# Luckick/EAGCN

Measured on AMD Instinct MI355X. Metric: molecules/sec fwd+bwd, 2-layer 5-view EAGCN, Tox21 batch, higher is better.
Workload: dtype f32 (bf16x3 split, fp32 accumulate): every fp32 operand leaves its producer as three bf16 planes, six v_mfma_f32_32x32x16_bf16 piece products per 16 k rebuild the fp32 product (csrc/gemm_bx3.hip); aggregation, BatchNorm, head, first layer fp32

## Files before the change

eagcn_amd/_lib.py:

```python
import ctypes as C
import os

_HERE = os.path.dirname(os.path.abspath(__file__))
LIB_PATH = os.path.join(_HERE, 'lib', 'libeagcn_hip.so')

MAX_VIEWS = 8
MAX_SEGS = 8
META_WORDS = 16
META_NLOG = 8
META_T, META_NMAX, META_NTILES, META_BAD_ADJ, META_BAD_REL, META_NEDGE, META_OVERFLOW, META_EDGE_OVERFLOW = range(8)
META_NBLK = 9
STRUCT_CONCATE, STRUCT_WEIGHTED = 0, 1

_fp = C.c_void_p


class Batch(C.Structure):
    _fields_ = [('B', C.c_int32), ('N', C.c_int32), ('K', C.c_int32), ('ldc', C.c_int32),
                ('T', C.c_int32), ('n_max', C.c_int32), ('n_tiles', C.c_int32),
                ('channels', C.c_int32 * MAX_VIEWS),
                ('code', _fp), ('deg_bn', _fp), ('nat', _fp), ('row0', _fp), ('tile0', _fp),
                ('meta', _fp), ('row_mol', _fp), ('row_loc', _fp), ('row_m', _fp), ('row_deg', _fp),
                ('tile_mol', _fp), ('row_info', _fp), ('tile_info', _fp),
                ('rel_vec', _fp * MAX_VIEWS), ('rel_c', C.c_int32 * MAX_VIEWS),
# ... 171 lines not shown
    'eagcn_index_build': (C.c_int, [_fp, C.POINTER(_fp), C.POINTER(Batch), _fp, _fp]),
    'eagcn_index_from_bonds': (C.c_int, [_fp, _fp, _fp, _fp, C.c_int64, C.POINTER(Batch), _fp, _fp]),
    'eagcn_index_rows': (C.c_int, [C.POINTER(Batch), _fp]),
    'eagcn_set_gemm_mode': (C.c_int, [C.c_int]),
    'eagcn_stream_wait_counter': (C.c_int, [_fp, C.c_uint32, _fp]),
    'eagcn_stream_signal_flag': (C.c_int, [_fp, _fp]),
    'eagcn_stream_wait_flag': (C.c_int, [_fp, C.c_double, _fp]),
    'eagcn_stream_wait_timeouts': (C.c_int, []),
    'eagcn_stream_wait_reset': (None, []),
    'eagcn_adam_step': (C.c_int, [_fp, _fp, _fp, _fp, C.c_int64, _fp, _fp, _fp, _fp]),
    'eagcn_grad_norm_workspace_bytes': (C.c_size_t, []),
    'eagcn_grad_norm': (C.c_int, [_fp, _fp, C.c_int64, _fp, C.c_int, _fp]),
    'eagcn_adam_step_clipped': (C.c_int, [_fp, _fp, _fp, _fp, C.c_int64, _fp, _fp, _fp, _fp, _fp, _fp, _fp]),
    'eagcn_agg_wants_bond_lists': (C.c_int, [C.c_int, C.c_int]),
    'eagcn_agg_wants_bond_lists_for': (C.c_int, [C.c_int, C.c_int, C.c_int]),
    'eagcn_bx3_used_splits': (C.c_int, [C.c_int, C.c_int, C.c_int, C.c_int]),
    'eagcn_set_bx3_wide': (C.c_int, [C.c_int]),
    'eagcn_set_top_bn_sums': (C.c_int, [C.c_int]),
    'eagcn_set_hidden_bn_sums': (C.c_int, [C.c_int]),
    'eagcn_hidden_bn_sums_taken': (C.c_long, [C.c_int]),
    'eagcn_set_first_layer_fused': (C.c_int, [C.c_int]),
    'eagcn_first_layer_fused_taken': (C.c_long, [C.c_int]),
    'eagcn_first_layer_fused_last': (None, [C.POINTER(C.c_int32)]),
    'eagcn_bx3_pair_used_splits': (C.c_int, [C.c_int] * 7),
    'eagcn_bx3_plane_elems': (C.c_size_t, [C.c_int, C.c_int]),
    'eagcn_bx3_split': (C.c_int, [_fp, C.c_int, C.c_int, _fp, C.c_size_t, C.c_int, C.c_int, _fp]),
    'eagcn_gemm_bx3': (C.c_int, [C.c_int, C.c_int, C.c_int, C.c_int, _fp, C.c_size_t, C.c_int, C.c_int, _fp, C.c_size_t, C.c_int, C.c_int,
                                 _fp, C.c_int, C.c_int, C.c_size_t, C.c_int, _fp]),
    'eagcn_gemm_bx3_pair': (C.c_int, [C.c_int, C.c_int, C.c_int, _fp, C.c_size_t, C.c_int, C.c_int, _fp, C.c_size_t, C.c_int, C.c_int, _fp, C.c_int,
                                      C.c_int, C.c_int, C.c_int, _fp, C.c_size_t, C.c_int, C.c_int, _fp, C.c_size_t, C.c_int, C.c_int, _fp, C.c_int,
                                      C.c_int, C.c_size_t, C.c_int, _fp]),
    'eagcn_pack_rows': (C.c_int, [C.POINTER(Batch), _fp, C.c_int, C.POINTER(Layout), _fp, _fp]),
    'eagcn_unpack_rows': (C.c_int, [C.POINTER(Batch), _fp, C.POINTER(Layout), _fp, _fp, C.c_int, _fp]),
    'eagcn_pad_rows': (C.c_int, [_fp, _fp, C.c_int, C.c_int, C.c_int, _fp, _fp]),
    'eagcn_gat_scratch_bytes': (C.c_size_t, [C.POINTER(Batch), C.c_int]),
    'eagcn_gat_forward': (C.c_int, [C.POINTER(Batch), C.POINTER(GatParams), _fp, _fp, _fp, _fp, _fp]),
    'eagcn_gat_backward': (C.c_int, [C.POINTER(Batch), C.POINTER(GatParams), _fp, _fp, _fp, _fp, _fp, _fp, _fp, _fp, _fp,
                                     C.c_size_t, _fp]),
    'eagcn_pool_scratch_bytes': (C.c_size_t, []),
    'eagcn_pool_attention_forward': (C.c_int, [C.POINTER(Batch), C.POINTER(PoolAtt), _fp, C.c_int, _fp, _fp, _fp]),
    'eagcn_pool_attention_backward': (C.c_int, [C.POINTER(Batch), C.POINTER(PoolAtt), _fp, C.c_int, _fp, _fp, _fp, C.c_size_t,
                                                _fp]),
    'eagcn_pool_mix_forward': (C.c_int, [C.POINTER(Batch), C.POINTER(Layout), _fp, C.c_int, _fp, _fp, _fp, _fp, C.c_int, _fp]),
    'eagcn_pool_mix_backward': (C.c_int, [C.POINTER(Batch), C.POINTER(Layout), _fp, C.c_int, _fp, _fp, _fp, _fp, C.c_int, _fp,
                                          _fp, _fp, _fp]),
    'eagcn_pool_reduce_forward': (C.c_int, [C.POINTER(Batch), _fp, C.c_int, C.c_int, C.c_int, _fp, _fp, _fp, _fp]),
# ... 157 lines not shown
```

eagcn_amd/build.py:

```python
import os
import shutil
import subprocess
import sys
from concurrent.futures import ThreadPoolExecutor

HERE = os.path.dirname(os.path.abspath(__file__))
CSRC = os.path.join(HERE, 'csrc')
LIBDIR = os.path.join(HERE, 'lib')
LIB = os.path.join(LIBDIR, 'libeagcn_hip.so')
HIP_SOURCES = ['index.hip', 'gemm.hip', 'gemm3.hip', 'gemm_bx3.hip', 'gemm_bx3w.hip', 'agg.hip', 'lagg.hip', 'lagg_in.hip', 'lagg_top.hip', 'lagg_dw.hip', 'gat.hip', 'pool.hip', 'layer.hip', 'readout.hip', 'head.hip', 'head2.hip', 'loss.hip', 'clip.hip', 'attr.hip', 'battr.hip', 'metrics.hip', 'reps.hip', 'embed.hip', 'knn.hip']
CPP_SOURCES = ['api.cpp']
HEADERS = ['common.h', 'kernels.h', 'lagg_kernel.h', 'gemm_x6.h', 'bx3.h', 'bx3_epi.h', os.path.join('..', '..', 'include', 'eagcn_hip.h')]
ARCH = 'gfx950'


def _hipcc():
    for cand in (shutil.which('hipcc'), '/opt/rocm/bin/hipcc'):
        if cand and os.path.exists(cand):
            return cand
    raise RuntimeError('hipcc not found: the EAGCN HIP library cannot be built')


def _newest(paths):
    return max(os.path.getmtime(p) for p in paths)


def needs_build():
    srcs = [os.path.join(CSRC, s) for s in HIP_SOURCES + CPP_SOURCES + HEADERS if os.path.exists(os.path.join(CSRC, s))]
    return (not os.path.exists(LIB)) or os.path.getmtime(LIB) < _newest(srcs)


def build_library(force=False, verbose=False):
    if not force and not needs_build():
# ... 38 lines not shown
```

eagcn_amd/csrc/kernels.h:

```cpp
#pragma once
#include "bx3.h"
#include "common.h"

namespace eagcn {

struct AggArgs {
    eagcn_batch bt;
    ViewCols vc;
    const float* src; int lds;
    float* dst; int ldd;
    const float* sig;
    const float* rsig;
    float* rscale;
    double* stats;
    int nchunk;
    int cpw = 1;
    int xcd = 0;
    bool w_rowm = false;
    bool w_gather = false;
    BxOut planes = {nullptr, 0, 0, 0};
    const float* bn_tab = nullptr; const float* bn_cc = nullptr; int bn_fp = 0;
    const float* w_aw = nullptr;
    int w_drop = 0; uint32_t w_thr = 0; float w_inv_keep = 1.0f; uint64_t w_seed = 0; const uint64_t* w_seed_dev = nullptr;
    const float* fx = nullptr; int fx_ld = 0; float* dw = nullptr; size_t dw_slab = 0; int dw_ny = 0;
};
struct DropArgs { int on; uint32_t thr; float inv_keep; uint64_t seed; const uint64_t* seed_dev; };
inline DropArgs drop_args(float p, bool training, uint64_t seed, const uint64_t* seed_dev) {
    const double thr = (double)p * 4294967296.0;
    return DropArgs{(training && p > 0.0f) ? 1 : 0, (uint32_t)(thr < 4294967295.0 ? thr : 4294967295.0), 1.0f / (1.0f - p), seed, seed_dev};
}
inline void agg_set_drop(AggArgs& a, const DropArgs& d) {
    a.w_drop = d.on; a.w_thr = d.thr; a.w_inv_keep = d.inv_keep; a.w_seed = d.seed; a.w_seed_dev = d.seed_dev;
}
int agg_grid_x(const eagcn_batch* b);
bool agg_ksplit(const eagcn_batch* b);
int launch_agg(AggArgs a, bool trans, hipStream_t s);
constexpr int LAGG_RB = 256;
constexpr int LAGG_MAXM = 16;
struct EdgeArgs;
int lagg_parts();
bool lagg_wfuse();
bool lagg_use(const eagcn_batch* b, int dir, bool absorbs_bn, const ViewCols* vc = nullptr);
bool lagg_wanted(int B, int N, int structure);
int lagg_block_rows(const eagcn_batch* b);
int lagg_slabs(const eagcn_batch* b);
int launch_lagg_fwd(AggArgs a, hipStream_t s);
int launch_lagg_bwd(AggArgs a, const EdgeArgs& e, hipStream_t s, bool edge = true);
int launch_lagg_bwd_input(const AggArgs& a, const EdgeArgs& e, dim3 grid, hipStream_t s);
int launch_lagg_bwd_top(const AggArgs& a, const EdgeArgs& e, dim3 grid, hipStream_t s);
int launch_lagg_bwd_dw(const AggArgs& a, const EdgeArgs& e, dim3 grid, hipStream_t s);
int lagg_bwd_grid_y(const eagcn_batch* b, const ViewCols& vc);

struct EdgeArgs {
    eagcn_batch bt;
    ViewCols vc;
    const float* dY; const float* Y; const float* P; int ld;
    const float* sig; const float* rsig; const float* rscale;
    double* datt;
    int atomic;
    int xcd = 0;
};
constexpr int EDGE_SLAB = 264;
constexpr int EDGE_COPIES = 8;
inline size_t edge_acc_bytes() { return align256((size_t)EDGE_COPIES * EAGCN_MAX_VIEWS * EDGE_SLAB * sizeof(double)); }
int edge_grid_x(const eagcn_batch* b);
int launch_agg_edge(AggArgs a, const EdgeArgs& e, hipStream_t s);

enum { BN_SC = 0, BN_SH, BN_MU, BN_INV };

struct ColMapD {
    int nseg;
    int w[EAGCN_MAX_SEGS], p[EAGCN_MAX_SEGS];
};
// ... 182 lines not shown
struct PlanAsk {
    bool has_dx = false;
    bool mol_grad = false;
    bool input_only = false;
    bool has_drain_out = false;
    bool top_sums = false;
    bool top_gather = false;
    bool dh_given = false;
    bool below = false;
};
struct LayerRoute {
    FwdProd fwd_prod = FWD_NONE; bool fwd_split_x = false;
    AggPath fwd_agg = AGG_DENSE, bwd_agg = AGG_DENSE;
    Bn2 bn2 = BN2_NONE;
    bool rows_first = false, rows_late = false;
    bool store_dh = false;
    EdgePath edge = EDGE_NONE; bool edge_atomic = false;
    BwdProd bwd_prod = BWD_NONE; bool bwd_split_x = false;
    bool bx_wide = false;
    bool carries_below = false;
    bool defer_drain = false;
    bool dh_given = false;
    bool dw_fused = false; int dw_ny = 0; bool dw_in_dp = false;
    bool bn2_staged() const { return bn2 >= BN2_STAGED_FROM_DH; }
    bool bwd_planes() const { return bwd_prod >= BWD_PLANES_PAIR && bwd_prod <= BWD_PLANES_DX; }
};
LayerRoute plan_layer(const eagcn_batch* b, const eagcn_layer_params* p, const eagcn_layer_bufs* w, const PlanAsk& ask);
int layer_backward_impl(const eagcn_batch* b, const eagcn_layer_params* p, const eagcn_layer_bufs* w, const float* dxout,
                        const float* dpad_row, float* dx, const eagcn_layer_grads* g, void* stream, const LayerRoute& r,
                        const LayerBwdOpts& o = LayerBwdOpts{});
int model_backward_input_packed(const eagcn_batch* b, const eagcn_model* m, const int64_t* size, void* saved, size_t saved_bytes,
                                void* scratch, size_t scratch_bytes, const float* dout, const float* dgraph_rep,
                                const eagcn_layer_grads* lg, const eagcn_head_grads* hg, float** dx0, void* stream, const char* who);
int launch_attr_dense(const eagcn_batch* b, const eagcn_layout* in, const float* acc, const float* x, const float* base, float* attr,
                      float* score, hipStream_t s);
int model_input_slot(const eagcn_batch* b, const eagcn_model* m, void* saved, size_t saved_bytes, float** x0, const char* who);
int layer_forward_impl(const eagcn_batch* b, const eagcn_layer_params* p, const eagcn_layer_bufs* w, void* stream, const LayerRoute& r,
                       bool prepacked, bool skip_apply = false, bool planes_only = false);
inline int check_reserved_null(const void* value, const char* who, const char* field) {
    EAGCN_CHECK_ARG(!value, "%s: %s is reserved and must be null", who, field);
    return EAGCN_OK;
}
int layer_apply_impl(const eagcn_batch* b, const eagcn_layer_params* p, const eagcn_layer_bufs* w, void* stream);
int pack_params_all(const eagcn_batch* b, const eagcn_layer_params* const* ps, void* const* packed,
                    const size_t* packed_bytes, int n, void* stream, const ZeroJob* zj = nullptr, const HandOff* ho = nullptr);
struct ReadoutBn {
// ... 22 lines not shown
```

eagcn_amd/csrc/lagg.hip:

```cpp
#include <stdlib.h>

#include <algorithm>

#include "common.h"
#include "kernels.h"
#include "lagg_kernel.h"

namespace eagcn {


static int lagg_cpw(const eagcn_batch& bt, const ViewCols& vc, bool trans);
static int lagg_policy() {
    static const int v = [] {
        const char* e = getenv("EAGCN_AGG");
        if (e && !strcmp(e, "lds")) return 1;
        if (e && !strcmp(e, "dense")) return 0;
        return 2;
    }();
    return v;
}
static int lagg_min_n() {
    static const int v = env_int("EAGCN_LAGG_MIN_N", 240);
    return v;
}
// ... 44 lines not shown
    static const int cpw_env = env_int("EAGCN_LAGG_CPW", 0);
    static const int cpw_bwd = env_int("EAGCN_LAGG_CPW_BWD", 1);
    int chunks, gy;
    lagg_extent(bt, vc, &chunks, &gy);
    const long wgs = (long)vc.K * chunks * gy;
    int per = (trans && !cpw_bwd) ? 1 : cpw_env > 0 ? cpw_env : (int)std::min<long>(trans ? 4 : 8, std::max<long>(1, wgs / 3072));
    return std::max(1, std::min(per, chunks));
}
static int lagg_grid(const AggArgs& a, dim3* grid, int* nchunk, int* cpw, bool trans) {
    int chunks, gy;
    lagg_extent(a.bt, a.vc, &chunks, &gy);
    *cpw = lagg_cpw(a.bt, a.vc, trans);
    *nchunk = cdiv(chunks, *cpw);
    *grid = dim3((unsigned)(a.vc.K * *nchunk), (unsigned)gy);
    return EAGCN_OK;
}

int lagg_bwd_grid_y(const eagcn_batch* b, const ViewCols& vc) {
    int chunks, gy;
    lagg_extent(*b, vc, &chunks, &gy);
    return gy;
}

int launch_lagg_fwd(AggArgs a, hipStream_t s) {
    if (a.bt.B == 0 || a.bt.T == 0) return EAGCN_OK;
    dim3 grid;
    int rc = lagg_grid(a, &grid, &a.nchunk, &a.cpw, false);
    if (rc) return rc;
    ProfScope ps(PROF_AGG, s);
    EdgeArgs e;
    memset(&e, 0, sizeof(e));
    if (a.cpw > 1) lagg_kernel<false, true><<<grid, 256, 0, s>>>(a, e);
    else lagg_kernel<false, false><<<grid, 256, 0, s>>>(a, e);
    EAGCN_LAUNCH_CHECK();
    return EAGCN_OK;
}

int launch_lagg_bwd(AggArgs a, const EdgeArgs& e, hipStream_t s, bool edge) {
    if (a.bt.B == 0 || a.bt.T == 0) return EAGCN_OK;
    EAGCN_CHECK_ARG(!edge || (e.atomic && e.datt), "lagg: the edge gradients leave through the shared accumulator slabs (EdgeArgs.atomic)");
    dim3 grid;
    int rc = lagg_grid(a, &grid, &a.nchunk, &a.cpw, true);
    if (rc) return rc;
    ProfScope ps(PROF_AGG, s);
    EAGCN_CHECK_ARG(!a.w_aw || a.bn_tab, "lagg: the upstream-gradient form needs the BatchNorm tables");
    EAGCN_CHECK_ARG(!a.w_rowm || a.bn_tab, "lagg: the row-mask staging needs the BatchNorm tables");
    if (!edge) {
        rc = launch_lagg_bwd_input(a, e, grid, s);
        if (rc) return rc;
    } else if (a.w_rowm) {
        rc = launch_lagg_bwd_top(a, e, grid, s);
        if (rc) return rc;
// ... 19 lines not shown
```

eagcn_amd/csrc/lagg_kernel.h:

```cpp
#pragma once

#include "common.h"
#include "kernels.h"

namespace eagcn {

constexpr int LG_CW = 32;
constexpr int LG_LPR = LG_CW / 4;
constexpr int LG_G = 256 / LG_LPR;
constexpr int LG_U = LAGG_RB / LG_G;
constexpr int LG_ECAP = 768;
constexpr int LG_EPT = LG_ECAP / 256;
constexpr bool LG_MERGE = true;
constexpr int LG_PJ_EARLY = 4;

__device__ __forceinline__ void lg_fma(float4& acc, float w, const float4& v) {
    acc.x = fmaf(w, v.x, acc.x); acc.y = fmaf(w, v.y, acc.y); acc.z = fmaf(w, v.z, acc.z); acc.w = fmaf(w, v.w, acc.w);
}
__device__ __forceinline__ void lg_add(float4& acc, const float4& v) { acc.x += v.x; acc.y += v.y; acc.z += v.z; acc.w += v.w; }
__device__ __forceinline__ float lg_dot(const float4& a, const float4& b) { return fmaf(a.x, b.x, fmaf(a.y, b.y, fmaf(a.z, b.z, a.w * b.w))); }
template <int CTRL>
__device__ __forceinline__ float lg_dpp(float v) {
    return __int_as_float(__builtin_amdgcn_update_dpp(0, __float_as_int(v), CTRL, 0xF, 0xF, true));
}
__device__ __forceinline__ float lg_gsum(float v) {
    v += lg_dpp<0xB1>(v); v += lg_dpp<0x4E>(v); v += lg_dpp<0x141>(v);
    return v;
}

struct LgLists {
    unsigned short nb[LG_ECAP];
    float w[LG_ECAP];
    unsigned char cd[LG_ECAP];
};
constexpr uint32_t LG_SLOW = 1u << 28;
constexpr uint32_t LG_OVF = 1u << 29;
constexpr int LG_NOVF = 32;

template <bool TRANS, bool MULTI, bool WFUSE = false, bool EDGE = true, bool CROWS = false, bool GATHER = false, bool DWF = false>
__global__ __launch_bounds__(256) __attribute__((amdgpu_waves_per_eu(3, 8))) void lagg_kernel(AggArgs a, EdgeArgs ed) {
    static_assert(!DWF || (TRANS && EDGE && !WFUSE), "the weight-gradient epilogue belongs to the plain transposed kernel with the edge gradients");
    static_assert(TRANS || !WFUSE, "the upstream-gradient form belongs to the transposed kernel");
    static_assert(TRANS || EDGE, "the forward has no edge gradients to drop");
    static_assert(!CROWS || WFUSE, "the row-mask staging is a form of the upstream-gradient staging");
    static_assert(!GATHER || (CROWS && EDGE && MULTI), "the per-molecule gather is a form of the row-mask staging with the edge gradients");
    constexpr bool TE = TRANS && EDGE;
    constexpr int NREC = TRANS ? 3 : 2;
    __shared__ float4 buf[LAGG_RB][LG_LPR];
    __shared__ float4 s_rec[LAGG_RB][NREC];
    __shared__ float4 s_ovf[LG_NOVF][NREC];
    __shared__ int s_novf;
    __shared__ __attribute__((aligned(16))) unsigned char s_lists_raw[TRANS ? 16 : sizeof(LgLists)];
    __shared__ float s_rs[TRANS ? LAGG_RB : 1];
    __shared__ float s_rd[TE ? LAGG_RB : 1];
    __shared__ unsigned char s_rm[LAGG_RB];
    __shared__ float4 s_S[LAGG_MAXM][LG_LPR];
    __shared__ float sig_s[256];
    __shared__ double st_s[TRANS ? 1 : 4][TRANS ? 1 : LG_LPR][8];
    __shared__ float4 s_bn[TRANS ? (WFUSE ? 4 : 3) : 1][LG_LPR];
    __shared__ double h_s[TE ? 264 : 1];
    static_assert(sizeof(LgLists) <= sizeof(float4) * LAGG_RB * 3, "lists alias the transposed record array");
    LgLists& L = *reinterpret_cast<LgLists*>(TRANS ? reinterpret_cast<unsigned char*>(&s_rec[0][0]) : s_lists_raw);
    const eagcn_batch& bt = a.bt;
    const int tid = threadIdx.x, lane = tid & 63, wave = tid >> 6;
// ... 200 lines not shown
#pragma unroll
                for (int i = 0; i < NREC; ++i) s_rec[tid][i] = rec[i];
            }
        };
        if constexpr (MULTI) {
            hdr_loads();
            if (nst > 0) list_loads();
            __syncthreads();
            lists_to_lds();
            __syncthreads();
            build_record();
            if constexpr (TRANS) __syncthreads();
            write_record();
        }
        for (int cc = cc_lo; cc < cc_hi; ++cc) {
        set_chunk(cc);
        asm volatile("" : "+v"(g));
        const bool bn_next = MULTI && TRANS && fuse_bn && tid < LG_CW;

        float4 v[LG_U], yv[TRANS ? LG_U : 1];
        float rmv[(CROWS && !EDGE) ? LG_U : 1];
        int ce = 0;
        if constexpr (GATHER) { const int cx = c0s - a.vc.off[k]; ce = ex0 + (cx < a.vc.width[k] ? cx : 0); }
#pragma unroll
        for (int u = 0; u < LG_U; ++u) {
            const int rc = min(g + LG_G * u, rows - 1);
            if constexpr (GATHER) v[u] = *reinterpret_cast<const float4*>(a.src + ((uint32_t)(m0 + s_rm[rc]) * (uint32_t)a.lds + (uint32_t)ce));
            else v[u] = *reinterpret_cast<const float4*>(a.src + (size_t)(R0 + rc) * a.lds + ((WFUSE && !CROWS) ? (col_ok ? col : 0) : c0s));
            if constexpr (TRANS) yv[u] = *reinterpret_cast<const float4*>(ed.Y + (size_t)(R0 + rc) * ed.ld + c0s);
            if constexpr (CROWS && !EDGE) rmv[u] = bt.row_m[R0 + rc];
        }
        if constexpr (!MULTI) {
            hdr_loads();
            if (nst > 0) list_loads();
        }
        uint32_t keep = 0xFFFFFFFFu;
        if constexpr (WFUSE) {
            if (a.w_drop) {
                keep = 0u;
                const uint32_t t16 = a.w_thr >> 16;
#pragma unroll
                for (int u = 0; u < LG_U; ++u) {
                    const uint64_t z = rng_u64(wseed, ((uint64_t)(R0 + g + LG_G * u) * a.bn_fp + c0s) >> 2);
                    const uint32_t lo = (uint32_t)z, hi = (uint32_t)(z >> 32);
                    keep |= ((lo & 0xFFFFu) >= t16 ? 1u : 0u) << (4 * u);
                    keep |= ((lo >> 16) >= t16 ? 2u : 0u) << (4 * u);
                    keep |= ((hi & 0xFFFFu) >= t16 ? 4u : 0u) << (4 * u);
                    keep |= ((hi >> 16) >= t16 ? 8u : 0u) << (4 * u);
                }
            }
        }
        __syncthreads();
        if (tid < LAGG_MAXM * LG_LPR) {
            float z;
            asm volatile("v_mov_b32 %0, 0" : "=v"(z));
            (&s_S[0][0])[tid] = make_float4(z, z, z, z);
        }
#pragma unroll
        for (int u = 0; u < LG_U; ++u) {
            const int rr = g + LG_G * u;
            const bool mine = rr < rows;
            if constexpr (TRANS) {
                if (fuse_bn) {
                    if constexpr (WFUSE) {
                        int lq = l;
                        asm volatile("" : "+v"(lq));
                        if constexpr (GATHER) {
                            if (c0s - a.vc.off[k] >= a.vc.width[k]) v[u] = make_float4(0.f, 0.f, 0.f, 0.f);
                        }
                        uint32_t mb;
                        {
                            const float4 bA = s_bn[0][lq], sh = s_bn[3][lq];
                            const uint32_t kb = keep >> (4 * u);
                            mb = ((yv[u].x * bA.x + sh.x > 0.0f) ? (kb & 1u) : 0u) | ((yv[u].y * bA.y + sh.y > 0.0f) ? (kb & 2u) : 0u) |
                                 ((yv[u].z * bA.z + sh.z > 0.0f) ? (kb & 4u) : 0u) | ((yv[u].w * bA.w + sh.w > 0.0f) ? (kb & 8u) : 0u);
                        }
                        asm volatile("" : "+v"(mb));
                        {
                            const float ik = a.w_drop ? a.w_inv_keep : 1.0f;
                            float wm = w_ave;
                            if constexpr (CROWS && !EDGE) wm = rmv[u];
                            if constexpr (CROWS && EDGE) wm = s_rs[rr] > 0.0f ? 1.0f : 0.0f;
// ... 136 lines not shown
            if constexpr (AHEAD) {
#pragma unroll
                for (int i = 0; i < NREC; ++i) nrec[i] = s_rec[min(g, rows - 1)][i];
            }
            const int nu = (rows + LG_G - 1) / LG_G;
#pragma unroll
            for (int u = 0; u < LG_U; ++u) {
                if (!DWF && u >= nu) break;
                const int rr = min(g + LG_G * u, rows - 1);
                const bool valid = g + LG_G * u < rows;
                if constexpr (!AHEAD) {
#pragma unroll
                    for (int i = 0; i < NREC; ++i) nrec[i] = s_rec[rr][i];
                }
                const float4 r0 = nrec[0], r1 = nrec[1], rl = nrec[NREC - 1];
                if (AHEAD && u + 1 < LG_U) {
#pragma unroll
                    for (int i = 0; i < NREC; ++i) nrec[i] = s_rec[min(rr + LG_G, rows - 1)][i];
                }
                const uint32_t srcs = __float_as_uint(TRANS ? rl.y : rl.z), meta = __float_as_uint(rl.w);
                const bool fast = valid && !(meta & LG_SLOW);
                any_slow = any_slow || (valid && (meta & LG_SLOW));
                const float4 self = buf[rr][l];
                const float4 S = s_S[(meta >> 24) & 15u][l];
                const float4 v0 = buf[srcs & 255u][l], v1 = buf[(srcs >> 8) & 255u][l], v2 = buf[(srcs >> 16) & 255u][l], v3 = buf[srcs >> 24][l];
                const float ws = TRANS ? r * rl.x : r1.x;
                const float wS = TRANS ? TINY : r1.y * TINY;
                float4 y;
                y.x = fmaf(r0.x, v0.x, fmaf(r0.y, v1.x, fmaf(r0.z, v2.x, fmaf(r0.w, v3.x, fmaf(ws, self.x, wS * S.x)))));
                y.y = fmaf(r0.x, v0.y, fmaf(r0.y, v1.y, fmaf(r0.z, v2.y, fmaf(r0.w, v3.y, fmaf(ws, self.y, wS * S.y)))));
                y.z = fmaf(r0.x, v0.z, fmaf(r0.y, v1.z, fmaf(r0.z, v2.z, fmaf(r0.w, v3.z, fmaf(ws, self.z, wS * S.z)))));
                y.w = fmaf(r0.x, v0.w, fmaf(r0.y, v1.w, fmaf(r0.z, v2.w, fmaf(r0.w, v3.w, fmaf(ws, self.w, wS * S.w)))));
                if constexpr (TE && LG_MERGE) {
                    const float4 pj = col_ok ? pjv[u] : make_float4(0.f, 0.f, 0.f, 0.f);
                    const uint32_t cds = __float_as_uint(rl.z);
                    const float g0 = lg_gsum(lg_dot(v0, pj)), g1 = lg_gsum(lg_dot(v1, pj)), g2 = lg_gsum(lg_dot(v2, pj)), g3 = lg_gsum(lg_dot(v3, pj));
                    const float gs = lg_gsum(lg_dot(self, pj));
                    const int e4 = l & 3;
                    const float hv = e4 == 0 ? r1.x : e4 == 1 ? r1.y : e4 == 2 ? r1.z : r1.w;
                    const float gv = e4 == 0 ? g0 : e4 == 1 ? g1 : e4 == 2 ? g2 : g3;
                    const uint32_t cv = (cds >> (8 * e4)) & 255u, sv = (srcs >> (8 * e4)) & 255u;
                    if (fast && l < 4 && hv != 0.0f && cv) atomicAdd(&h_s[cv], (double)hv * ((double)gv - (double)s_rd[sv]));
                    if (fast && l == 4) dr_acc += (double)rl.x * ((double)gs - (double)s_rd[rr]);
                }
                if (fast && (meta & LG_OVF)) {
                    const int slot = (int)(meta & 0xFFFFu);
// ... 177 lines not shown
```

eagcn_amd/csrc/layer.hip:

```cpp
#include <algorithm>

#include <stdlib.h>

#include "common.h"
#include "kernels.h"

namespace eagcn {

struct ParamPtrs {
    const float* att_w[EAGCN_MAX_VIEWS];
    const float* self_r[EAGCN_MAX_VIEWS];
    const float* W[EAGCN_MAX_VIEWS];
    const float* bias[EAGCN_MAX_VIEWS];
    const float* gamma[EAGCN_MAX_VIEWS];
    const float* beta[EAGCN_MAX_VIEWS];
    float* run_mean[EAGCN_MAX_VIEWS];
    float* run_var[EAGCN_MAX_VIEWS];
    const float* ave_w;
    int channels[EAGCN_MAX_VIEWS];
    const float* rel_vec[EAGCN_MAX_VIEWS];
    int rel_c[EAGCN_MAX_VIEWS];
};
__device__ __forceinline__ float att_logit(const ParamPtrs& pp, int k, int c) {
    if (!pp.rel_vec[k]) return pp.att_w[k][c - 1];
// ... 849 lines not shown
static Fp32Products layer_fp32_products(const eagcn_batch* b, const LayerDims& d, const LayerOperands& o, double work) {
    const int* T_dev = b->meta + EAGCN_META_T;
    Fp32Products q{GemmDesc{0, 1, b->T, d.fp, d.ld_in, o.x, d.ld_in, o.pk.WcatT, d.ld_in, o.P, d.fp, 1, 0, work},
                   GemmDesc{0, 0, b->T, d.fp, d.ld_in, o.x, d.ld_in, o.pk.Wcat, d.fp, o.P, d.fp, 1, 0, work},
                   GemmDesc{0, 1, b->T, d.ld_in, d.fp, o.dP, d.fp, o.pk.Wcat, d.fp, o.dx, d.ld_in, 1, 0, work},
                   GemmDesc{1, 0, d.ld_in, d.fp, b->T, o.x, d.ld_in, o.dP, d.fp, o.dWcat, d.fp, d.nsplit, d.wslab, work}};
    q.gp.M_dev = T_dev; q.gt.M_dev = T_dev; q.gx.M_dev = T_dev; q.gw.K_dev = T_dev;
    return q;
}

static bool sw_gemm3() { static const bool on = !env_flag("EAGCN_NO_GEMM3", false); return on; }
bool planes_only_enabled() { static const bool on = env_flag("EAGCN_PLANES_ONLY", true); return on; }
static bool bn_bwd_two_pass(bool weighted) {
    static const int force = getenv("EAGCN_BWD_STORE_DH") ? (env_flag("EAGCN_BWD_STORE_DH", false) ? 1 : 0) : -1;
    return force < 0 ? weighted : force == 0;
}
static bool gemm3_layer(int ld_in) {
    return sw_gemm3() && ld_in >= 128 && gemm_mode() != 2;
}
static int g_first_layer_fused = env_flag("EAGCN_FIRST_LAYER_FUSED", true) ? 1 : 0;
static long g_first_layer_fused_taken = 0;
static int32_t g_first_layer_fused_last[3] = {0, 0, 0};
static bool first_layer_fused_enabled() { return g_first_layer_fused != 0; }
static int g_hidden_bn_sums = env_flag("EAGCN_HIDDEN_BN_SUMS", true) ? 1 : 0;
static long g_hidden_bn_taken = 0;

static LayerRoute plan_layer(const eagcn_batch* b, const eagcn_layer_params* p, const eagcn_layer_bufs* w, const LayerDims& d,
                             const PlanAsk& ask) {
    LayerRoute r;
    const bool wt = p->structure == EAGCN_STRUCT_WEIGHTED;
    bool general = false;
    for (int k = 0; k < p->K; ++k) general = general || b->rel_vec[k] != nullptr;
    r.edge_atomic = !general;
    r.store_dh = !bn_bwd_two_pass(wt);
    if (b->T <= 0) return r;
    r.fwd_agg = fwd_agg_lagg(b, d.vc) ? AGG_LAGG : AGG_DENSE;
    float* const some_dx = reinterpret_cast<float*>(static_cast<uintptr_t>(4096));
    LayerScratch sc;
    carve_layer(w->scratch, b, d, true, &sc);
    if (w->packed) carve_packed(w->packed, d, &sc.pk);
    const LayerOperands o = layer_operands(w, sc, ask.has_dx ? some_dx : nullptr);
    const PlaneProducts bq = layer_plane_products(b, d, o);
    const Fp32Products gq = layer_fp32_products(b, d, o, 0.0);

    r.fwd_split_x = d.np && !w->x_planes;
    if (d.np && bx3_ok(bq.bp)) r.fwd_prod = FWD_PLANES;
    else if (!w->x) r.fwd_prod = FWD_REFUSED;
    else r.fwd_prod = (gemm3_layer(d.ld_in) && gemm3_ok(gq.gp)) ? FWD_BALANCED : FWD_TILED;

    const bool fuse_w = bn_bwd_two_pass(wt) && wt && lagg_wfuse();
    const bool absorbs = !bn_bwd_two_pass(wt) || (wt && lagg_wfuse());
    const bool lagg = ask.input_only ? lagg_use(b, 1, true) : (r.edge_atomic && lagg_use(b, 1, absorbs));
    r.bwd_agg = lagg ? AGG_LAGG : AGG_DENSE;
    if (ask.input_only && !p->training) {
        r.bn2 = !lagg ? BN2_REDUCE_APPLY : wt ? BN2_STAGED_FROM_UPSTREAM : BN2_STAGED_ROWMASK;
        r.rows_first = lagg && ask.mol_grad;
    } else if (lagg && fuse_w) {
        r.bn2 = BN2_STAGED_FROM_UPSTREAM;
        r.rows_first = ask.mol_grad;
    } else if (bn_bwd_two_pass(wt)) r.bn2 = BN2_REDUCE_APPLY;
    else r.bn2 = lagg ? BN2_STAGED_FROM_DH : BN2_ELEMENTWISE;
    if (ask.top_sums && r.bn2 == BN2_STAGED_FROM_DH && ask.mol_grad && !wt) {
        r.bn2 = BN2_STAGED_FROM_READOUT;
        r.rows_late = !ask.top_gather;
        r.store_dh = false;
    }

    r.dh_given = ask.dh_given && g_hidden_bn_sums && r.bn2 == BN2_STAGED_FROM_DH && r.store_dh && !wt && p->training && !ask.mol_grad &&
                 !ask.input_only && hidden_bn_slabs(b->T) <= d.gxb;
    const bool planes = d.np && bx3_ok(bq.bw) && (!ask.has_dx || bx3_ok(bq.bx));
    r.bwd_split_x = planes && !w->x_planes && !ask.input_only;
// ... 166 lines not shown
    EAGCN_CHECK_ARG(!prepacked || w->packed, "eagcn_layer_forward: prepacked parameters need the packed block");
    if (!prepacked) launch_pack_params(pp, d, make_colmap(&p->in), sc.pk, s);
    EAGCN_LAUNCH_CHECK();
    int nslab = 0, tiles_per_wg = agg_ksplit(b) ? 1 : 4;
    if (b->T > 0) {
        const double gemm_work = layer_gemm_work(b, p, d);
        const LayerOperands o = layer_operands(w, sc, nullptr);
        const Fp32Products gq = layer_fp32_products(b, d, o, gemm_work);
        if (r.fwd_prod == FWD_REFUSED) {
            set_error("eagcn_layer_forward: the input exists as plane images only and the plane product does not apply");
            return EAGCN_ERR_ARG;
        }
        if (r.fwd_split_x) {
            rc = launch_bx3_split(w->x, b->T, b->meta + EAGCN_META_T, d.ld_in, sc.xp, bx_plane_elems(b->T, d.ld_in), b->T, d.np, s);
            if (rc) return rc;
        }
        switch (r.fwd_prod) {
        case FWD_PLANES: {
            const BxProb bp = layer_plane_products(b, d, o).bp;
            rc = launch_bx3(bp, nullptr, d.np, s, gemm_work, PROF_GEMM, bx3_pick_wide(bp, nullptr, b->t_hint));
            break;
        }
        case FWD_BALANCED: rc = launch_gemm3(gq.gp, nullptr, sc.gws, gemm3_workspace_bytes(), s); break;
        default: rc = launch_gemm(gq.gt, s); break;
        }
        if (rc) return rc;
        AggArgs a;
        a.bt = *b; a.vc = d.vc; a.src = w->P; a.lds = d.fp; a.dst = w->Y; a.ldd = d.fp;
        a.sig = sc.pk.sig; a.rsig = sc.pk.rsig; a.rscale = w->rscale; a.stats = sc.stats; a.nchunk = 1;
        if (r.fwd_agg == AGG_LAGG) {
            rc = launch_lagg_fwd(a, s);
            nslab = lagg_slabs(b);
            tiles_per_wg = -1;
        } else {
            rc = launch_agg(a, false, s);
            nslab = d.gx;
        }
        if (rc) return rc;
    }
    const double M = (double)b->B * (double)b->N;
    {
        ProfScope psbn(PROF_BN, s);
        const bool sync = w->stats_hook && p->training;
        if (sync) {
            EAGCN_BY_SLABS(nslab, bn_stats_sum_kernel, sc.stats, nslab, d.fp, M, sc.gsum, b->meta, 1, tiles_per_wg, 0, b->B);
            EAGCN_LAUNCH_CHECK();
            if (w->stats_hook(sc.gsum, 2 * d.fp + 1, stream, w->stats_user)) {
                set_error("eagcn_layer_forward: the sync-BatchNorm all-reduce hook failed");
                return EAGCN_ERR_HIP;
            }
            nslab = 1;
        }
        EAGCN_BY_SLABS(nslab, bn_finalize_kernel, sync ? sc.gsum : sc.stats, nslab, d.fp, M, p->training, p->bn_eps, p->bn_momentum, sc.pk.colp,
                       pp, d.vc, w->bn, b->meta, sync ? 0 : tiles_per_wg, b->B, sync ? sc.gsum + 2 * d.fp : nullptr);
        EAGCN_LAUNCH_CHECK();
    }
    if (skip_apply) return EAGCN_OK;
    return apply_launch(b, p, w, d, sc.pk.colp, s, planes_only);
}

static int g_top_bn_sums = !env_flag("EAGCN_TOP_BN_SUMS", true) ? 0 : env_int("EAGCN_TOP_BN_SUMS", 1) == 2 ? 2 : 1;
// ... 4 lines not shown
    g_top_bn_sums = on == 2 ? 2 : on ? 1 : 0;
    return old;
}
extern "C" long eagcn_hidden_bn_sums_taken(int reset) {
    const long n = g_hidden_bn_taken;
    if (reset) g_hidden_bn_taken = 0;
    return n;
}
extern "C" int eagcn_set_hidden_bn_sums(int on) {
    const int old = g_hidden_bn_sums;
    g_hidden_bn_sums = on ? 1 : 0;
    return old;
}
extern "C" long eagcn_first_layer_fused_taken(int reset) {
    const long n = g_first_layer_fused_taken;
    if (reset) g_first_layer_fused_taken = 0;
    return n;
}
extern "C" void eagcn_first_layer_fused_last(int32_t out[3]) { memcpy(out, g_first_layer_fused_last, sizeof(g_first_layer_fused_last)); }
extern "C" int eagcn_set_first_layer_fused(int on) {
    const int old = g_first_layer_fused;
    g_first_layer_fused = on ? 1 : 0;
    return old;
}
int eagcn::layer_apply_impl(const eagcn_batch* b, const eagcn_layer_params* p, const eagcn_layer_bufs* w, void* stream) {
    EAGCN_CHECK_ARG(b && p && w && w->bn && w->xout && w->pad_row && w->packed, "layer_apply: null buffer");
    const LayerDims d = layer_dims(b, p);
    Packed pk;
    EAGCN_CHECK_ARG(carve_packed(w->packed, d, &pk) <= w->packed_bytes, "layer_apply: packed buffer too small");
    return apply_launch(b, p, w, d, pk.colp, (hipStream_t)stream);
}

static void launch_bn_bwd_pass(bool apply, bool wt, bool dg, bool dr, dim3 grid, const BwdArgs& ba, hipStream_t s) {
#define EAGCN_BWD(W, G, D) do { if (apply) bn_bwd_reduce_kernel<W, G, D, true><<<grid, 256, 0, s>>>(ba); \
                                else bn_bwd_reduce_kernel<W, G, D, false><<<grid, 256, 0, s>>>(ba); } while (0)
    if (wt) { if (dg) { if (dr) EAGCN_BWD(true, true, true); else EAGCN_BWD(true, true, false); }
              else    { if (dr) EAGCN_BWD(true, false, true); else EAGCN_BWD(true, false, false); } }
    else    { if (dg) { if (dr) EAGCN_BWD(false, true, true); else EAGCN_BWD(false, true, false); }
              else    { if (dr) EAGCN_BWD(false, false, true); else EAGCN_BWD(false, false, false); } }
#undef EAGCN_BWD
}

extern "C" int eagcn_layer_backward(const eagcn_batch* b, const eagcn_layer_params* p, const eagcn_layer_bufs* w,
                                    const float* dxout, const float* dpad_row, float* dx,
                                    const eagcn_layer_grads* g, void* stream) {
    EAGCN_CHECK_GEMM3("eagcn_layer_backward");
// ... 314 lines not shown
```

include/eagcn_hip.h:

```cpp
#ifndef EAGCN_HIP_H
#define EAGCN_HIP_H

#include <stddef.h>
#include <stdint.h>

#ifdef __cplusplus
extern "C" {
#endif

#define EAGCN_MAX_VIEWS 8
#define EAGCN_MAX_SEGS 8
#define EAGCN_MAX_CHANNELS 255
#define EAGCN_STRUCT_CONCATE 0
#define EAGCN_STRUCT_WEIGHTED 1

#define EAGCN_OK 0
#define EAGCN_ERR_ARG (-1)
#define EAGCN_ERR_HIP (-2)
#define EAGCN_ERR_SCRATCH (-3)

#define EAGCN_META_T 0
#define EAGCN_META_NMAX 1
#define EAGCN_META_NTILES 2
#define EAGCN_META_BAD_ADJ 3
// ... 344 lines not shown
int eagcn_pca_cov(const float* X, int64_t n, int F, int ld, double* mean, double* cov, void* workspace, size_t workspace_bytes, void* stream);
int eagcn_pca_project(const float* X, int64_t n, int F, int ld, const double* mean, const float* components, int k, float* out,
                      void* stream);

#define EAGCN_KNN_MAX_K 128
size_t eagcn_knn_workspace_bytes(int64_t n, int64_t m, int F, int k, int slabs);
int eagcn_knn(const float* X, int64_t n, int F, int ldx, const float* Q, int64_t m, int ldq, int k, int exclude_self, int slabs,
              int32_t* idx, float* dist, void* ws, size_t ws_bytes, void* stream);
int eagcn_knn_rank(const float* X, int64_t n, int F, int ld, const int32_t* cand, int k, int slabs, int32_t* rank, void* ws,
                   size_t ws_bytes, void* stream);

int eagcn_set_gemm_mode(int mode);

size_t eagcn_bx3_plane_elems(int rows_cap, int ld);
int eagcn_bx3_split(const float* x, int rows, int ld, uint16_t* planes, size_t plane_stride, int rows_cap, int np, void* stream);
int eagcn_bx3_used_splits(int splits, int M, int N, int K);
int eagcn_set_bx3_wide(int mode);
int eagcn_set_top_bn_sums(int on);
int eagcn_set_hidden_bn_sums(int on);
long eagcn_hidden_bn_sums_taken(int reset);
int eagcn_set_first_layer_fused(int on);
long eagcn_first_layer_fused_taken(int reset);
void eagcn_first_layer_fused_last(int32_t out[3]);
int eagcn_bx3_pair_used_splits(int splits, int M, int N, int K, int M0, int N0, int K0);
int eagcn_gemm_bx3(int tn, int M, int N, int K, const uint16_t* A, size_t a_pstride, int lda, int a_rows, const uint16_t* B,
                   size_t b_pstride, int ldb, int b_rows, float* C, int ldc, int splits, size_t slab, int np, void* stream);
int eagcn_gemm_bx3_pair(int M0, int N0, int K0, const uint16_t* A0, size_t a0_pstride, int lda0, int a0_rows, const uint16_t* B0,
                        size_t b0_pstride, int ldb0, int b0_rows, float* C0, int ldc0, int M1, int N1, int K1, const uint16_t* A1,
                        size_t a1_pstride, int lda1, int a1_rows, const uint16_t* B1, size_t b1_pstride, int ldb1, int b1_rows,
                        float* C1, int ldc1, int splits, size_t slab, int np, void* stream);

int eagcn_gemm_f32(int ta, int tb, int M, int N, int K, const float* A, int lda, const float* B,
                   int ldb, float* C, int ldc, void* stream);
int eagcn_gemm_f32_dev(int ta, int tb, int M, int N, int K, const float* A, int lda, const float* B,
                       int ldb, float* C, int ldc, const int32_t* extent_dev, int which, void* stream);

size_t eagcn_gemm_sk_workspace_bytes(void);
int eagcn_gemm_f32_sk(int ta, int tb, int M, int N, int K, const float* A, int lda, const float* B, int ldb, float* C,
                      int ldc, void* workspace, size_t workspace_bytes, void* stream);
int eagcn_gemm_pair_sk(int M0, int N0, int K0, const float* A0, int lda0, const float* B0, int ldb0, float* C0, int ldc0,
                       int M1, int N1, int K1, const float* A1, int lda1, const float* B1, int ldb1, float* C1, int ldc1,
                       void* workspace, size_t workspace_bytes, void* stream);
int eagcn_gemm_pair_sk_slabs(int M0, int N0, int K0, const float* A0, int lda0, const float* B0, int ldb0, float* C0, int ldc0,
                             int M1, int N1, int K1, const float* A1, int lda1, const float* B1, int ldb1, float* C1, int ldc1,
                             size_t slab, void* workspace, size_t workspace_bytes, void* stream);
int eagcn_gemm_sk_plan(int M0, int N0, int K0, int M1, int N1, int K1, int wgs, int* a, int* c);
// ... 16 lines not shown
```

Baseline: 781,700.

## Fuse first-layer forward projection GEMM into the aggregation kernel staging

For the first layer (input width ≤32, tiled fp32 GEMM route, lagg aggregation), the separate GEMM that produces P = x·W is skipped. The aggregation kernel instead loads the input rows, computes the projection in shared memory with fp32 MFMA 16x16x4, writes P out for the backward pass, and aggregates from the staged product. This removes one kernel launch and the write-then-read round trip of P before aggregation. In exchange the aggregation kernel carries extra register and shared-memory pressure and repeats the projection per column chunk.

```diff
diff --git a/eagcn_amd/_lib.py b/eagcn_amd/_lib.py
--- a/eagcn_amd/_lib.py
+++ b/eagcn_amd/_lib.py
@@ -217,6 +217,10 @@
     'eagcn_set_first_layer_fused': (C.c_int, [C.c_int]),
     'eagcn_first_layer_fused_taken': (C.c_long, [C.c_int]),
     'eagcn_first_layer_fused_last': (None, [C.POINTER(C.c_int32)]),
+    'eagcn_set_first_layer_fwd_fused': (C.c_int, [C.c_int]),
+    'eagcn_first_layer_fwd_fused_taken': (C.c_long, [C.c_int]),
+    'eagcn_first_layer_fwd_fused_last': (None, [C.POINTER(C.c_int32)]),
+    'eagcn_layer_fwd_in_agg': (C.c_int, [C.POINTER(Batch), C.POINTER(LayerParams), C.POINTER(LayerBufs)]),
     'eagcn_bx3_pair_used_splits': (C.c_int, [C.c_int] * 7),
     'eagcn_bx3_plane_elems': (C.c_size_t, [C.c_int, C.c_int]),
     'eagcn_bx3_split': (C.c_int, [_fp, C.c_int, C.c_int, _fp, C.c_size_t, C.c_int, C.c_int, _fp]),
diff --git a/eagcn_amd/build.py b/eagcn_amd/build.py
--- a/eagcn_amd/build.py
+++ b/eagcn_amd/build.py
@@ -8,7 +8,7 @@
 CSRC = os.path.join(HERE, 'csrc')
 LIBDIR = os.path.join(HERE, 'lib')
 LIB = os.path.join(LIBDIR, 'libeagcn_hip.so')
-HIP_SOURCES = ['index.hip', 'gemm.hip', 'gemm3.hip', 'gemm_bx3.hip', 'gemm_bx3w.hip', 'agg.hip', 'lagg.hip', 'lagg_in.hip', 'lagg_top.hip', 'lagg_dw.hip', 'gat.hip', 'pool.hip', 'layer.hip', 'readout.hip', 'head.hip', 'head2.hip', 'loss.hip', 'clip.hip', 'attr.hip', 'battr.hip', 'metrics.hip', 'reps.hip', 'embed.hip', 'knn.hip']
+HIP_SOURCES = ['index.hip', 'gemm.hip', 'gemm3.hip', 'gemm_bx3.hip', 'gemm_bx3w.hip', 'agg.hip', 'lagg.hip', 'lagg_in.hip', 'lagg_top.hip', 'lagg_dw.hip', 'lagg_fx.hip', 'gat.hip', 'pool.hip', 'layer.hip', 'readout.hip', 'head.hip', 'head2.hip', 'loss.hip', 'clip.hip', 'attr.hip', 'battr.hip', 'metrics.hip', 'reps.hip', 'embed.hip', 'knn.hip']
 CPP_SOURCES = ['api.cpp']
 HEADERS = ['common.h', 'kernels.h', 'lagg_kernel.h', 'gemm_x6.h', 'bx3.h', 'bx3_epi.h', os.path.join('..', '..', 'include', 'eagcn_hip.h')]
 ARCH = 'gfx950'
diff --git a/eagcn_amd/csrc/kernels.h b/eagcn_amd/csrc/kernels.h
--- a/eagcn_amd/csrc/kernels.h
+++ b/eagcn_amd/csrc/kernels.h
@@ -23,6 +23,7 @@
     const float* w_aw = nullptr;
     int w_drop = 0; uint32_t w_thr = 0; float w_inv_keep = 1.0f; uint64_t w_seed = 0; const uint64_t* w_seed_dev = nullptr;
     const float* fx = nullptr; int fx_ld = 0; float* dw = nullptr; size_t dw_slab = 0; int dw_ny = 0;
+    const float* fxw = nullptr; float* p_out = nullptr;
 };
 struct DropArgs { int on; uint32_t thr; float inv_keep; uint64_t seed; const uint64_t* seed_dev; };
 inline DropArgs drop_args(float p, bool training, uint64_t seed, const uint64_t* seed_dev) {
@@ -44,11 +45,12 @@
 bool lagg_wanted(int B, int N, int structure);
 int lagg_block_rows(const eagcn_batch* b);
 int lagg_slabs(const eagcn_batch* b);
-int launch_lagg_fwd(AggArgs a, hipStream_t s);
+int launch_lagg_fwd(AggArgs a, hipStream_t s, int* cpw_out = nullptr);
 int launch_lagg_bwd(AggArgs a, const EdgeArgs& e, hipStream_t s, bool edge = true);
 int launch_lagg_bwd_input(const AggArgs& a, const EdgeArgs& e, dim3 grid, hipStream_t s);
 int launch_lagg_bwd_top(const AggArgs& a, const EdgeArgs& e, dim3 grid, hipStream_t s);
 int launch_lagg_bwd_dw(const AggArgs& a, const EdgeArgs& e, dim3 grid, hipStream_t s);
+int launch_lagg_fwd_fx(const AggArgs& a, dim3 grid, hipStream_t s);
 int lagg_bwd_grid_y(const eagcn_batch* b, const ViewCols& vc);
 
 struct EdgeArgs {
@@ -277,6 +279,7 @@
     bool defer_drain = false;
     bool dh_given = false;
     bool dw_fused = false; int dw_ny = 0; bool dw_in_dp = false;
+    bool fwd_in_agg = false;
     bool bn2_staged() const { return bn2 >= BN2_STAGED_FROM_DH; }
     bool bwd_planes() const { return bwd_prod >= BWD_PLANES_PAIR && bwd_prod <= BWD_PLANES_DX; }
 };
diff --git a/eagcn_amd/csrc/lagg.hip b/eagcn_amd/csrc/lagg.hip
--- a/eagcn_amd/csrc/lagg.hip
+++ b/eagcn_amd/csrc/lagg.hip
@@ -90,12 +90,15 @@
     return gy;
 }
 
-int launch_lagg_fwd(AggArgs a, hipStream_t s) {
+int launch_lagg_fwd(AggArgs a, hipStream_t s, int* cpw_out) {
+    if (cpw_out) *cpw_out = 0;
     if (a.bt.B == 0 || a.bt.T == 0) return EAGCN_OK;
     dim3 grid;
     int rc = lagg_grid(a, &grid, &a.nchunk, &a.cpw, false);
     if (rc) return rc;
+    if (cpw_out) *cpw_out = a.cpw;
     ProfScope ps(PROF_AGG, s);
+    if (a.p_out) return launch_lagg_fwd_fx(a, grid, s);
     EdgeArgs e;
     memset(&e, 0, sizeof(e));
     if (a.cpw > 1) lagg_kernel<false, true><<<grid, 256, 0, s>>>(a, e);
diff --git a/eagcn_amd/csrc/lagg_fx.hip b/eagcn_amd/csrc/lagg_fx.hip
--- /dev/null
+++ b/eagcn_amd/csrc/lagg_fx.hip
@@ -0,0 +1,22 @@
+#include <stdint.h>
+
+#include "lagg_kernel.h"
+
+namespace eagcn {
+
+int launch_lagg_fwd_fx(const AggArgs& a, dim3 grid, hipStream_t s) {
+    EAGCN_CHECK_ARG(a.fx && a.fxw && a.p_out, "lagg: the forward with the product in its staging needs the layer's input, its packed weight and P");
+    EAGCN_CHECK_ARG(a.fx_ld >= 4 && a.fx_ld <= LG_CW && (a.fx_ld & 3) == 0,
+                    "lagg: the forward with the product in its staging takes 4..32 input columns, a multiple of four (%d)", a.fx_ld);
+    EAGCN_CHECK_ARG(((reinterpret_cast<uintptr_t>(a.fx) | reinterpret_cast<uintptr_t>(a.fxw) | reinterpret_cast<uintptr_t>(a.p_out)) & 15) == 0 &&
+                        (a.lds & 3) == 0,
+                    "lagg: the forward with the product in its staging needs 16-byte aligned operands");
+    EdgeArgs e;
+    memset(&e, 0, sizeof(e));
+    if (a.cpw > 1) lagg_kernel<false, true, false, true, false, false, false, true><<<grid, 256, 0, s>>>(a, e);
+    else lagg_kernel<false, false, false, true, false, false, false, true><<<grid, 256, 0, s>>>(a, e);
+    EAGCN_LAUNCH_CHECK();
+    return EAGCN_OK;
+}
+
+}
diff --git a/eagcn_amd/csrc/lagg_kernel.h b/eagcn_amd/csrc/lagg_kernel.h
--- a/eagcn_amd/csrc/lagg_kernel.h
+++ b/eagcn_amd/csrc/lagg_kernel.h
@@ -37,9 +37,11 @@
 constexpr uint32_t LG_OVF = 1u << 29;
 constexpr int LG_NOVF = 32;
 
-template <bool TRANS, bool MULTI, bool WFUSE = false, bool EDGE = true, bool CROWS = false, bool GATHER = false, bool DWF = false>
+template <bool TRANS, bool MULTI, bool WFUSE = false, bool EDGE = true, bool CROWS = false, bool GATHER = false, bool DWF = false,
+          bool FXF = false>
 __global__ __launch_bounds__(256) __attribute__((amdgpu_waves_per_eu(3, 8))) void lagg_kernel(AggArgs a, EdgeArgs ed) {
     static_assert(!DWF || (TRANS && EDGE && !WFUSE), "the weight-gradient epilogue belongs to the plain transposed kernel with the edge gradients");
+    static_assert(!FXF || (!TRANS && !DWF), "the product in the staging belongs to the forward kernel");
     static_assert(TRANS || !WFUSE, "the upstream-gradient form belongs to the transposed kernel");
     static_assert(TRANS || EDGE, "the forward has no edge gradients to drop");
     static_assert(!CROWS || WFUSE, "the row-mask staging is a form of the upstream-gradient staging");
@@ -286,8 +288,33 @@
         float rmv[(CROWS && !EDGE) ? LG_U : 1];
         int ce = 0;
         if constexpr (GATHER) { const int cx = c0s - a.vc.off[k]; ce = ex0 + (cx < a.vc.width[k] ? cx : 0); }
-#pragma unroll
-        for (int u = 0; u < LG_U; ++u) {
+        constexpr int FX_KS = LG_CW / 4;
+        float wb[FXF ? FX_KS : 1][FXF ? 2 : 1];
+        if constexpr (FXF) {
+            const int li = lane & 15, kq = lane >> 4;
+            const uint32_t fp = (uint32_t)a.vc.off[a.vc.K];
+            uint32_t cb[2];
+#pragma unroll
+            for (int j = 0; j < 2; ++j) {
+                const int cv = cc * LG_CW + 16 * j + li;
+                cb[j] = (uint32_t)(a.vc.off[k] + (cv < wk ? cv : 0));
+            }
+            const uint32_t xc = (uint32_t)min(4 * l, a.fx_ld - 4);
+#pragma unroll
+            for (int u = 0; u < LG_U; ++u)
+                v[u] = *reinterpret_cast<const float4*>(a.fx + ((uint32_t)(R0 + min(g + LG_G * u, rows - 1)) * (uint32_t)a.fx_ld + xc));
+#pragma unroll
+            for (int ks = 0; ks < FX_KS; ++ks) {
+                wb[ks][0] = wb[ks][1] = 0.0f;
+                if (4 * ks < a.fx_ld) {
+                    const uint32_t kk = (uint32_t)(4 * ks + kq) * fp;
+#pragma unroll
+                    for (int j = 0; j < 2; ++j) wb[ks][j] = a.fxw[kk + cb[j]];
+                }
+            }
+        }
+#pragma unroll
+        for (int u = 0; u < (FXF ? 0 : LG_U); ++u) {
             const int rc = min(g + LG_G * u, rows - 1);
             if constexpr (GATHER) v[u] = *reinterpret_cast<const float4*>(a.src + ((uint32_t)(m0 + s_rm[rc]) * (uint32_t)a.lds + (uint32_t)ce));
             else v[u] = *reinterpret_cast<const float4*>(a.src + (size_t)(R0 + rc) * a.lds + ((WFUSE && !CROWS) ? (col_ok ? col : 0) : c0s));
@@ -320,8 +347,52 @@
             asm volatile("v_mov_b32 %0, 0" : "=v"(z));
             (&s_S[0][0])[tid] = make_float4(z, z, z, z);
         }
-#pragma unroll
-        for (int u = 0; u < LG_U; ++u) {
+        if constexpr (FXF) {
+            typedef float lg_fx4 __attribute__((ext_vector_type(4)));
+            const int li = lane & 15, kq = lane >> 4;
+#pragma unroll
+            for (int u = 0; u < LG_U; ++u) {
+                const int rr = g + LG_G * u;
+                if (rr < rows) buf[rr][l ^ (rr & 7)] = 4 * l < a.fx_ld ? v[u] : make_float4(0.f, 0.f, 0.f, 0.f);
+            }
+            __syncthreads();
+            float* bf = reinterpret_cast<float*>(&buf[0][0]);
+#pragma unroll 1
+            for (int h = 0; h < 2; ++h) {
+                lg_fx4 acc[2][2];
+                int xo[2];
+#pragma unroll
+                for (int i = 0; i < 2; ++i) {
+                    xo[i] = min(64 * wave + 32 * h + 16 * i + li, rows - 1);
+#pragma unroll
+                    for (int j = 0; j < 2; ++j) acc[i][j] = lg_fx4{0.f, 0.f, 0.f, 0.f};
+                }
+#pragma unroll
+                for (int ks = 0; ks < FX_KS; ++ks) {
+                    if (4 * ks < a.fx_ld) {
+#pragma unroll
+                        for (int i = 0; i < 2; ++i) {
+                            const float av = bf[xo[i] * LG_CW + 4 * (ks ^ (xo[i] & 7)) + kq];
+                            acc[i][0] = __builtin_amdgcn_mfma_f32_16x16x4f32(av, wb[ks][0], acc[i][0], 0, 0, 0);
+                            acc[i][1] = __builtin_amdgcn_mfma_f32_16x16x4f32(av, wb[ks][1], acc[i][1], 0, 0, 0);
+                        }
+                    }
+                }
+#pragma unroll
+                for (int j = 0; j < 2; ++j) {
+                    const bool cok = cc * LG_CW + 16 * j + li < wk;
+#pragma unroll
+                    for (int i = 0; i < 2; ++i)
+#pragma unroll
+                        for (int r4 = 0; r4 < 4; ++r4) {
+                            const int row = 64 * wave + 32 * h + 16 * i + 4 * kq + r4;
+                            if (row < rows) bf[row * LG_CW + 16 * j + li] = cok ? acc[i][j][r4] : 0.0f;
+                        }
+                }
+            }
+        }
+#pragma unroll
+        for (int u = 0; u < (FXF ? 0 : LG_U); ++u) {
             const int rr = g + LG_G * u;
             const bool mine = rr < rows;
             if constexpr (TRANS) {
@@ -504,6 +575,9 @@
                 const bool fast = valid && !(meta & LG_SLOW);
                 any_slow = any_slow || (valid && (meta & LG_SLOW));
                 const float4 self = buf[rr][l];
+                if constexpr (FXF) {
+                    if (valid && col_ok) *reinterpret_cast<float4*>(a.p_out + (size_t)(R0 + rr) * a.lds + c0) = self;
+                }
                 const float4 S = s_S[(meta >> 24) & 15u][l];
                 const float4 v0 = buf[srcs & 255u][l], v1 = buf[(srcs >> 8) & 255u][l], v2 = buf[(srcs >> 16) & 255u][l], v3 = buf[srcs >> 24][l];
                 const float ws = TRANS ? r * rl.x : r1.x;
diff --git a/eagcn_amd/csrc/layer.hip b/eagcn_amd/csrc/layer.hip
--- a/eagcn_amd/csrc/layer.hip
+++ b/eagcn_amd/csrc/layer.hip
@@ -895,6 +895,9 @@
 static long g_first_layer_fused_taken = 0;
 static int32_t g_first_layer_fused_last[3] = {0, 0, 0};
 static bool first_layer_fused_enabled() { return g_first_layer_fused != 0; }
+static int g_first_layer_fwd_fused = env_flag("EAGCN_FIRST_LAYER_FWD_FUSED", true) ? 1 : 0;
+static long g_first_layer_fwd_fused_taken = 0;
+static int32_t g_first_layer_fwd_fused_last[2] = {0, 0};
 static int g_hidden_bn_sums = env_flag("EAGCN_HIDDEN_BN_SUMS", true) ? 1 : 0;
 static long g_hidden_bn_taken = 0;
 
@@ -920,6 +923,9 @@
     if (d.np && bx3_ok(bq.bp)) r.fwd_prod = FWD_PLANES;
     else if (!w->x) r.fwd_prod = FWD_REFUSED;
     else r.fwd_prod = (gemm3_layer(d.ld_in) && gemm3_ok(gq.gp)) ? FWD_BALANCED : FWD_TILED;
+    const bool fx_aligned = ((reinterpret_cast<uintptr_t>(w->x) | reinterpret_cast<uintptr_t>(w->P)) & 15) == 0;
+    r.fwd_in_agg = g_first_layer_fwd_fused != 0 && r.fwd_prod == FWD_TILED && r.fwd_agg == AGG_LAGG && d.ld_in <= 32 && gemm_mode() != 1 &&
+                   gemm_mode() != 2 && w->x && fx_aligned;
 
     const bool fuse_w = bn_bwd_two_pass(wt) && wt && lagg_wfuse();
     const bool absorbs = !bn_bwd_two_pass(wt) || (wt && lagg_wfuse());
@@ -1132,14 +1138,16 @@
             break;
         }
         case FWD_BALANCED: rc = launch_gemm3(gq.gp, nullptr, sc.gws, gemm3_workspace_bytes(), s); break;
-        default: rc = launch_gemm(gq.gt, s); break;
+        default: rc = r.fwd_in_agg ? EAGCN_OK : launch_gemm(gq.gt, s); break;
         }
         if (rc) return rc;
         AggArgs a;
         a.bt = *b; a.vc = d.vc; a.src = w->P; a.lds = d.fp; a.dst = w->Y; a.ldd = d.fp;
         a.sig = sc.pk.sig; a.rsig = sc.pk.rsig; a.rscale = w->rscale; a.stats = sc.stats; a.nchunk = 1;
+        int fx_cpw = 0;
+        if (r.fwd_in_agg) { a.src = nullptr; a.fx = w->x; a.fx_ld = d.ld_in; a.fxw = sc.pk.Wcat; a.p_out = w->P; }
         if (r.fwd_agg == AGG_LAGG) {
-            rc = launch_lagg_fwd(a, s);
+            rc = launch_lagg_fwd(a, s, &fx_cpw);
             nslab = lagg_slabs(b);
             tiles_per_wg = -1;
         } else {
@@ -1147,6 +1155,10 @@
             nslab = d.gx;
         }
         if (rc) return rc;
+        if (r.fwd_in_agg) {
+            ++g_first_layer_fwd_fused_taken;
+            g_first_layer_fwd_fused_last[0] = fx_cpw; g_first_layer_fwd_fused_last[1] = d.ld_in;
+        }
     }
     const double M = (double)b->B * (double)b->N;
     {
@@ -1197,6 +1209,22 @@
     const int old = g_first_layer_fused;
     g_first_layer_fused = on ? 1 : 0;
     return old;
+}
+extern "C" long eagcn_first_layer_fwd_fused_taken(int reset) {
+    const long n = g_first_layer_fwd_fused_taken;
+    if (reset) g_first_layer_fwd_fused_taken = 0;
+    return n;
+}
+extern "C" void eagcn_first_layer_fwd_fused_last(int32_t out[2]) { memcpy(out, g_first_layer_fwd_fused_last, sizeof(g_first_layer_fwd_fused_last)); }
+extern "C" int eagcn_set_first_layer_fwd_fused(int on) {
+    const int old = g_first_layer_fwd_fused;
+    g_first_layer_fwd_fused = on ? 1 : 0;
+    return old;
+}
+extern "C" int eagcn_layer_fwd_in_agg(const eagcn_batch* b, const eagcn_layer_params* p, const eagcn_layer_bufs* w) {
+    LayerRoute r;
+    const int rc = plan_checked(b, p, w, PlanAsk{}, "eagcn_layer_fwd_in_agg", &r);
+    return rc ? -abs(rc) : (r.fwd_in_agg ? 1 : 0);
 }
 int eagcn::layer_apply_impl(const eagcn_batch* b, const eagcn_layer_params* p, const eagcn_layer_bufs* w, void* stream) {
     EAGCN_CHECK_ARG(b && p && w && w->bn && w->xout && w->pad_row && w->packed, "layer_apply: null buffer");
diff --git a/include/eagcn_hip.h b/include/eagcn_hip.h
--- a/include/eagcn_hip.h
+++ b/include/eagcn_hip.h
@@ -390,6 +390,10 @@
 int eagcn_set_first_layer_fused(int on);
 long eagcn_first_layer_fused_taken(int reset);
 void eagcn_first_layer_fused_last(int32_t out[3]);
+int eagcn_set_first_layer_fwd_fused(int on);
+long eagcn_first_layer_fwd_fused_taken(int reset);
+void eagcn_first_layer_fwd_fused_last(int32_t out[2]);
+int eagcn_layer_fwd_in_agg(const eagcn_batch* b, const eagcn_layer_params* p, const eagcn_layer_bufs* w);
 int eagcn_bx3_pair_used_splits(int splits, int M, int N, int K, int M0, int N0, int K0);
 int eagcn_gemm_bx3(int tn, int M, int N, int K, const uint16_t* A, size_t a_pstride, int lda, int a_rows, const uint16_t* B,
                    size_t b_pstride, int ldb, int b_rows, float* C, int ldc, int splits, size_t slab, int np, void* stream);
```

Result: no change. 800,600, median of 3 (+2.4%).
